# hawkn/emqx

Measured on AMD Instinct MI355X. Metric: topic matches/sec at 10M filters, higher is better.
Workload: dtype u8/u32; 1 GPU; c3: 10M mixed-wildcard filters incl. $share groups and '$SYS' exclusion; filters=10000002, topics_per_gpu_step=1000000, global_batch=1000000, parallelism=topic-sharded x1 (trie replicated), streams=3, distinct_batches=4, table_copies=1, outputs=pairs

## Files before the change

emqx_amd/build.py:

```python
from __future__ import annotations

import os
import subprocess
from pathlib import Path

PKG = Path(__file__).resolve().parent
ROOT = PKG.parent
CSRC = PKG / "csrc"

LIB_TMATCH = PKG / "libtmatch.so"
LIB_WORK = PKG / "libtmwork.so"
LIB_BENCH = PKG / "libtmbench.so"
LIB_ORACLE = ROOT / "oracle" / "liboracle.so"

ARCH = os.environ.get("TM_OFFLOAD_ARCH", "gfx950")


KERNEL_SOURCES = ("tm_kernels.hip", "tm_host.cpp", "tm_layout.h", "tm_dev.h")


def source_hash() -> str:
    import hashlib
    h = hashlib.sha256()
    for name in KERNEL_SOURCES:
        h.update(name.encode())
        h.update((CSRC / name).read_bytes())
    return h.hexdigest()[:16]


def _stale(out: Path, deps) -> bool:
    if not out.exists():
        return True
    t = out.stat().st_mtime
    return any(Path(d).stat().st_mtime > t for d in deps)


def _run(cmd, cwd=None):
    r = subprocess.run(cmd, cwd=cwd, capture_output=True, text=True)
    if r.returncode != 0:
        raise RuntimeError(f"build failed: {' '.join(map(str, cmd))}\n{r.stdout}\n{r.stderr}")


def build_tmatch(force: bool = False) -> Path:
    srcs = [CSRC / "tm_host.cpp", CSRC / "tm_kernels.hip"]
    deps = srcs + [CSRC / "tm_layout.h", CSRC / "tm_dev.h", ROOT / "include" / "tmatch.h"]
    if force or _stale(LIB_TMATCH, deps):
        tmp = LIB_TMATCH.with_suffix(".so.tmp")
        _run(["hipcc", "-O3", "-std=c++17", f"--offload-arch={ARCH}", "-fPIC", "-shared",
              "-Wall", "-Wno-unused-function", "-o", str(tmp)] + [str(s) for s in srcs])
        os.replace(tmp, LIB_TMATCH)
    return LIB_TMATCH


def build_variant(name: str, kernel_src: str | None = None, force: bool = False,
                  host_src: str | None = None) -> Path:
    out = PKG / "variants" / f"libtmatch_{name}.so"
    out.parent.mkdir(exist_ok=True)
    kern = Path(kernel_src) if kernel_src else CSRC / "tm_kernels.hip"
    srcs = [Path(host_src) if host_src else CSRC / "tm_host.cpp", kern]
    deps = srcs + [CSRC / "tm_layout.h", CSRC / "tm_dev.h", ROOT / "include" / "tmatch.h"]
    if force or _stale(out, deps):
        _run(["hipcc", "-O3", "-std=c++17", f"--offload-arch={ARCH}", "-fPIC", "-shared", "-Wall",
              "-Wno-unused-function", f"-I{CSRC}", "-o", str(out)] + [str(s) for s in srcs])
    return out


def build_work(force: bool = False) -> Path:
    src = CSRC / "workload.cpp"
    if force or _stale(LIB_WORK, [src]):
        tmp = LIB_WORK.with_suffix(".so.tmp")
        _run(["g++", "-O2", "-std=c++17", "-fPIC", "-shared", "-pthread", "-o", str(tmp), str(src)])
        os.replace(tmp, LIB_WORK)
    return LIB_WORK


def build_bench(force: bool = False) -> Path:
    src = CSRC / "hostbench.cpp"
    if force or _stale(LIB_BENCH, [src, ROOT / "include" / "tmatch.h"]):
        tmp = LIB_BENCH.with_suffix(".so.tmp")
        _run(["hipcc", "-O2", "-std=c++17", "-fPIC", "-shared", "-pthread", "-o", str(tmp), str(src), "-ldl"])
        os.replace(tmp, LIB_BENCH)
    return LIB_BENCH


def build_oracle(force: bool = False) -> Path:
    src = ROOT / "oracle" / "tm_oracle.c"
    if force or _stale(LIB_ORACLE, [src]):
        _run(["make", "-B" if force else "-s", "liboracle.so"], cwd=ROOT / "oracle")
    return LIB_ORACLE


def build_all(force: bool = False) -> None:
    build_tmatch(force)
    build_work(force)
    build_bench(force)
    build_oracle(force)


if __name__ == "__main__":
    build_all(force=True)
    print("built", LIB_TMATCH, LIB_WORK, LIB_ORACLE)
```

emqx_amd/csrc/tm_kernels.hip:

```cpp
#include "tm_dev.h"

#if defined(__HIP_DEVICE_COMPILE__) && !defined(__gfx950__)
#error "tm_kernels.hip: the tail tickets' ordering is argued for gfx950 only (see above)"
#endif

namespace tmx {


__device__ __forceinline__ uint4 ld4(const void *p) { return *reinterpret_cast<const uint4 *>(p); }
__device__ __forceinline__ uint4 ld4_once(const void *p) {
    typedef unsigned int u32x4 __attribute__((ext_vector_type(4)));
    const u32x4 v = __builtin_nontemporal_load(reinterpret_cast<const u32x4 *>(p));
    return make_uint4(v.x, v.y, v.z, v.w);
}

__device__ __forceinline__ uint32_t bloom_bit(const uint4 &n2, const uint4 &n3, uint32_t b) {
    const uint32_t j = b >> 5;
    const uint32_t w = j == 0 ? n2.z : j == 1 ? n2.w : j == 2 ? n3.x : j == 3 ? n3.y : j == 4 ? n3.z : n3.w;
    return (w >> (b & 31)) & 1u;
}

__device__ __forceinline__ uint32_t child_maybe(const DevIndex &ix, const uint4 &n1, const uint4 &n2, const uint4 &n3,
                                                uint32_t w, uint32_t h) {
    if ((n1.y & NLIT_MASK) >= WIDE_LIT)
        return n2.z == NONE ? 1u : w < ix.wcap ? (ix.wbits[n2.z + (w >> 5)] >> (w & 31)) & 1u : 0u;
    return bloom_bit(n2, n3, child_bit(h));
}

__device__ __forceinline__ bool child_alive(uint32_t lo, uint32_t hi, uint32_t lq, uint32_t L, uint32_t wq,
                                            uint32_t wq2) {
    const uint64_t m = (uint64_t)hi << 32 | lo;
    constexpr uint32_t AT_END = PSUM_HASH | PSUM_EXACT | PSUM_HDESC;
    if (lq == L) return (m & AT_END) != 0;
    if (m & PSUM_HASH) return true;
    if (wq != NONE && ((m >> (PSUM_BQ + psum_bit(child_hash(wq)))) & 1u)) return true;
    if (!(m & PSUM_PLUS)) return false;
    const uint32_t qq = (uint32_t)(m >> PSUM_QQ) & 15u;
    if (lq + 1 == L) return (qq & AT_END) != 0;
    if (qq & (PSUM_HASH | PSUM_PLUS)) return true;
    return wq2 != NONE && ((m >> (PSUM_BQQ + psum_bit(child_hash(wq2)))) & 1u);
}

__device__ __forceinline__ void pin(uint32_t &v) { asm volatile("" : "+v"(v)); }
__device__ __forceinline__ void pin(uint2 &v) { pin(v.x); pin(v.y); }
__device__ __forceinline__ void pin(uint4 &v) { pin(v.x); pin(v.y); pin(v.z); pin(v.w); }

struct WordAcc {
    uint32_t len, b0, b1;
    uint64_t start;
    __device__ __forceinline__ void reset(uint64_t s) {
        len = 0; b0 = b1 = 0; start = s;
    }
    __device__ __forceinline__ void push(uint32_t c) {
        uint32_t v = c << ((len & 3) * 8);
        if (len < 4) b0 |= v; else if (len < 8) b1 |= v;
        len++;
    }
};

struct GlobalSrc {
    const uint8_t *g;
    __device__ __forceinline__ uint4 ld16(uint64_t p) const { return ld4_once(g + p); }
    __device__ __forceinline__ uint32_t byte(uint64_t p) const { return g[p]; }
};
struct StagedSrc {
    const uint8_t *g;
    const uint4 *lds;
    uint64_t b0;
    bool staged;
    __device__ __forceinline__ uint4 ld16(uint64_t p) const {
        return staged ? lds[(uint32_t)(p - b0) >> 4] : ld4_once(g + p);
    }
    __device__ __forceinline__ uint32_t byte(uint64_t p) const {
        return staged ? reinterpret_cast<const uint8_t *>(lds)[(uint32_t)(p - b0)] : g[p];
    }
};

template <class Src>
__device__ bool bytes_eq(const uint8_t *a, const Src &src, uint64_t b, uint32_t n) {
    for (uint32_t i = 0; i < n; i++) if (a[i] != src.byte(b + i)) return false;
    return true;
}

template <class Src>
__device__ __forceinline__ uint64_t word_hash_dev(const WordAcc &w, const Src &src) {
    if (w.len <= VINL) return word_hash_short(w.b0, w.b1, w.len);
    uint64_t h = FNV_OFF;
    for (uint32_t i = 0; i < w.len; i++) h = (h ^ src.byte(w.start + i)) * FNV_PRIME;
    return word_hash_finish(h, w.len);
}

template <class Src>
__device__ uint32_t vocab_probe(const DevIndex &ix, uint32_t slot, uint32_t tag, uint32_t len, uint32_t b0,
                                uint32_t b1, const Src &src, uint64_t start) {
    for (;;) {
        const uint4 e = ld4(ix.vocab + slot);
        if (e.y == NONE) return NONE;
        if (e.x == tag) {
            if (len <= VINL) {
                if (e.z == b0 && e.w == b1) return e.y;
            } else if (e.w == len && bytes_eq(ix.wpool + e.z, src, start, len)) {
                return e.y;
            }
        }
        slot = (slot + 1) & ix.vmask;
    }
}

__device__ uint32_t vocab_probe_short(const DevIndex &ix, uint32_t slot, uint32_t tag, uint32_t b0, uint32_t b1) {
    for (;;) {
        const uint4 e = ld4(ix.vocab + slot);
        if (e.y == NONE) return NONE;
        if (e.x == tag && e.z == b0 && e.w == b1) return e.y;
        slot = (slot + 1) & ix.vmask;
    }
}

template <class Src>
__device__ uint32_t vocab_find(const DevIndex &ix, const WordAcc &w, const Src &src) {
    const uint64_t h = word_hash_dev(w, src);
    return vocab_probe(ix, (uint32_t)h & ix.vmask, vocab_tag(h, w.len), w.len, w.b0, w.b1, src, w.start);
}

__device__ __forceinline__ uint32_t ctab_find(const DevIndex &ix, uint32_t off, uint32_t mask, uint32_t wid,
                                              uint32_t h, uint32_t &slo, uint32_t &shi) {
    for (uint32_t s = h & mask;; s = (s + 1) & mask) {
        uint4 e = ld4(ix.ctab + off + s);
        pin(e);
        if (e.x == wid) { slo = e.z; shi = e.w; return e.y; }
        if (e.x == NONE) return NONE;
    }
}


template <int ML, bool LITE = false>
struct LdsStore {
    static constexpr uint32_t maxl = ML;
    static constexpr bool deferred = true;
    static constexpr bool cuts = ML > FAST_L;
    static constexpr bool need = ML > FAST_L || LITE;
    uint32_t *wid, *pend;
    uint8_t *len8;
    uint32_t stride;
    uint64_t mask;
    uint32_t pm;
    __device__ __forceinline__ void down(uint32_t l, bool via_plus) {
        if constexpr (cuts) pm = via_plus ? pm | (1u << l) : pm & ~(1u << l);
    }
    __device__ __forceinline__ void popped(uint32_t l) {
        if constexpr (cuts) pm &= (1u << (l - 1)) - 1u;
    }
    __device__ __forceinline__ void cut(uint32_t) {
        if constexpr (cuts) mask &= pm ? (1ull << (33u - __clz(pm))) - 1ull : 0ull;
    }
    __device__ __forceinline__ uint32_t get_wid(uint32_t l) const { return wid[l * stride]; }
    __device__ __forceinline__ void set_wid(uint32_t l, uint32_t w) { wid[l * stride] = w; }
    __device__ __forceinline__ void reset() { mask = 0; pm = 0; }
    __device__ __forceinline__ void put_word(uint32_t l, uint32_t b0, uint32_t b1, uint32_t len) {
        wid[l * stride] = b0; pend[l * stride] = b1; len8[l * stride] = (uint8_t)len;
    }
    __device__ __forceinline__ uint32_t word_b0(uint32_t l) const { return wid[l * stride]; }
    __device__ __forceinline__ uint32_t word_b1(uint32_t l) const { return pend[l * stride]; }
    __device__ __forceinline__ uint32_t word_len(uint32_t l) const { return len8[l * stride]; }
    __device__ __forceinline__ void push(uint32_t l, uint32_t node) {
        pend[l * stride] = node; mask |= 1ull << l;
    }
    __device__ __forceinline__ bool pop(uint32_t &l, uint32_t &node) {
        if (!mask) return false;
        l = 63u - (uint32_t)__clzll(mask);
        mask &= ~(1ull << l);
        node = pend[l * stride];
        return true;
    }
};

struct GlobalStore {
    static constexpr uint32_t maxl = MAX_LEVELS;
    static constexpr bool deferred = false;
    static constexpr bool cuts = true;
    static constexpr bool need = true;
    uint32_t *wid;
    uint2 *stk;
    uint8_t *plus_at;
    uint32_t top;
    __device__ __forceinline__ uint32_t get_wid(uint32_t l) const { return wid[l]; }
    __device__ __forceinline__ void set_wid(uint32_t l, uint32_t w) { wid[l] = w; }
    __device__ __forceinline__ void reset() { top = 0; }
    __device__ __forceinline__ void down(uint32_t l, bool via_plus) { plus_at[l] = via_plus; }
    __device__ __forceinline__ void popped(uint32_t l) { plus_at[l - 1] = 0; }
    __device__ void cut(uint32_t L) {
        int64_t q = (int64_t)L - 1;
        while (q >= 0 && !plus_at[q]) q--;
        while (top && (int64_t)stk[top - 1].x > q + 1) top--;
    }
    __device__ __forceinline__ void push(uint32_t l, uint32_t node) { stk[top++] = make_uint2(l, node); }
    __device__ __forceinline__ bool pop(uint32_t &l, uint32_t &node) {
        if (!top) return false;
        uint2 e = stk[--top]; l = e.x; node = e.y;
        return true;
    }
};


enum { RC_OK = 0, RC_BADARG = 1, RC_DEEP = 2 };

constexpr uint32_t VGROUP = 6;

template <class Src>
__device__ __noinline__ uint32_t count_slashes(const Src src, uint64_t p, uint64_t end) {
    uint32_t n = 0;
    for (; p < end; p += 64) {
        uint4 v[4];
#pragma unroll
        for (int c = 0; c < 4; c++) v[c] = p + 16 * c < end ? src.ld16(p + 16 * c) : make_uint4(0, 0, 0, 0);
#pragma unroll
        for (int c = 0; c < 4; c++) {
            const uint32_t w[4] = {v[c].x, v[c].y, v[c].z, v[c].w};
            const uint64_t q = p + 16 * c;
            const int k1 = q >= end ? 0 : end - q < 16 ? (int)(end - q) : 16;
#pragma unroll
            for (int j = 0; j < 4; j++) {
                const uint32_t x = w[j] ^ 0x2F2F2F2Fu;
                uint32_t nz = (((x & 0x7F7F7F7Fu) + 0x7F7F7F7Fu) | x) & 0x80808080u;
                const int valid = k1 - 4 * j;
                if (valid < 4) nz |= valid <= 0 ? 0x80808080u : 0x80808080u << (8 * valid);
                n += 4 - __popc(nz);
            }
        }
    }
    return n;
}

template <class S, class Src>
__device__ int tokenize(const DevIndex &ix, const Src &src, uint64_t beg, uint64_t end, S &st,
                        uint32_t &L, bool &dollar, uint64_t &xh, bool &all_found) {
    uint64_t longmask = 0;
    all_found = true; dollar = false; xh = FNV_OFF;
    const uint64_t p0 = beg & ~15ull;
    const uint4 z = make_uint4(0, 0, 0, 0);
    const uint4 c0 = p0 < end ? src.ld16(p0) : z;
    const uint4 c1 = p0 + 16 < end ? src.ld16(p0 + 16) : z;
    if constexpr (S::deferred) {
        constexpr bool NEED = S::need;
        uint32_t lev = 0, len = 0, b0 = 0, b1 = 0;
        uint64_t ws = beg;
        bool bad = false;
        auto park = [&]() {
            if (lev < S::maxl) {
                if (len <= VINL) st.put_word(lev, b0, b1, len);
                else st.put_word(lev, len, (uint32_t)(ws - beg), 255);
            } else if constexpr (NEED) {
                bad |= len == 1 && ((b0 & 0xFFu) == '+' || (b0 & 0xFFu) == '#');
            }
            lev++;
        };
        uint32_t ci = 0;
        uint64_t p = p0;
        uint4 ra = c0, rb = c1;
        for (; p < end; p += 16, ci++) {
            if (!NEED && lev > S::maxl) break;
            uint4 v;
            if constexpr (NEED) {
                v = ra; ra = rb;
                rb = p + 32 < end ? src.ld16(p + 32) : z;
            } else {
                v = ci == 0 ? c0 : ci == 1 ? c1 : src.ld16(p);
            }
            const uint32_t k0 = p < beg ? (uint32_t)(beg - p) : 0;
            const uint32_t k1 = end - p < 16 ? (uint32_t)(end - p) : 16;
#pragma unroll
            for (uint32_t k = 0; k < 16; k++) {
                if (k < k0 || k >= k1) continue;
                const uint32_t word = k < 4 ? v.x : k < 8 ? v.y : k < 12 ? v.z : v.w;
                const uint32_t c = (word >> ((k & 3) * 8)) & 0xFFu;
                if (c == '/') {
                    park();
                    len = 0; b0 = 0; b1 = 0; ws = p + k + 1;
                } else {
                    const uint32_t sh = (len & 3) * 8;
                    b0 |= len < 4 ? c << sh : 0u;
                    b1 |= len - 4 < 4 ? c << sh : 0u;
                    len++;
                }
            }
        }
        if (!NEED && p < end) {
            const bool any = ix.xlen_max <= S::maxl && ix.depth + 2 <= (uint32_t)MID_L &&
                             end - beg < (uint64_t)MAX_LEVELS;
            L = any ? lev + 1 : lev + 1 + count_slashes(src, p, end);
            return RC_DEEP;
        }
        park();
        if (lev > (NEED ? MAX_LEVELS : S::maxl)) { L = lev; return RC_DEEP; }
        L = lev;
        for (uint32_t l = 0; l < L && l < S::maxl; l++) {
            const uint32_t n = st.word_len(l), c = st.word_b0(l) & 0xFFu;
            bad |= n == 1 && (c == '+' || c == '#');
        }
        if (bad) return RC_BADARG;
        if constexpr (NEED) {
            const uint32_t Lw = need_levels(ix, L);
            if (Lw + (Lw < L ? 2 : 0) > S::maxl) return RC_DEEP;
            L |= Lw << 24;
        }
        dollar = st.word_len(0) == 255 ? src.byte(beg) == '$' : st.word_len(0) >= 1 && (st.word_b0(0) & 0xFFu) == '$';
        for (uint32_t l = 0; l < (S::need ? L >> 24 : L); l++) {
            if (st.word_len(l) != 255) continue;
            WordAcc w; w.reset(beg + st.word_b1(l)); w.len = st.word_b0(l);
            st.set_wid(l, vocab_find(ix, w, src));
            longmask |= 1ull << l;
        }
    } else {
        WordAcc w; w.reset(beg);
        uint32_t lev = 0;
        auto finish = [&]() -> int {
            if (w.len == 1 && (w.b0 == '+' || w.b0 == '#')) return RC_BADARG;
            if (lev >= S::maxl) return RC_DEEP;
            if (lev == 0 && w.len >= 1 && (w.b0 & 0xFF) == '$') dollar = true;
            st.set_wid(lev, vocab_find(ix, w, src));
            lev++;
            return RC_OK;
        };
        uint32_t ci = 0;
        for (uint64_t p = p0; p < end; p += 16, ci++) {
            const uint4 v = ci == 0 ? c0 : ci == 1 ? c1 : src.ld16(p);
            const uint32_t k0 = p < beg ? (uint32_t)(beg - p) : 0;
            const uint32_t k1 = end - p < 16 ? (uint32_t)(end - p) : 16;
            for (uint32_t k = k0; k < k1; k++) {
                const uint32_t word = k < 4 ? v.x : k < 8 ? v.y : k < 12 ? v.z : v.w;
                const uint32_t c = (word >> ((k & 3) * 8)) & 0xFFu;
                if (c == '/') {
                    int rc = finish();
                    if (rc) return rc;
                    w.reset(p + k + 1);
                } else {
                    w.push(c);
                }
            }
        }
        int rc = finish();
        if (rc) return rc;
        L = lev;
    }
    if constexpr (S::deferred) {
        for (uint32_t base = 0; base < (S::need ? L >> 24 : L); base += VGROUP) {
            uint4 e[VGROUP];
            uint32_t tg[VGROUP];
            bool use[VGROUP];
#pragma unroll
            for (uint32_t k = 0; k < VGROUP; k++) {
                const uint32_t l = base + k;
                use[k] = l < (S::need ? L >> 24 : L) && !((longmask >> l) & 1);
                const uint32_t ls = use[k] ? l : 0;
                const uint32_t len = st.word_len(ls);
                const uint64_t h = word_hash_short(st.word_b0(ls), st.word_b1(ls), len);
                tg[k] = vocab_tag(h, len);
                e[k] = ld4(ix.vocab + (use[k] ? ((uint32_t)h & ix.vmask) : 0u));
            }
#pragma unroll
            for (uint32_t k = 0; k < VGROUP; k++) {
                const uint32_t l = use[k] ? base + k : 0;
                const uint32_t b0 = st.word_b0(l), b1 = st.word_b1(l);
                const bool hit = e[k].x == tg[k] && e[k].z == b0 && e[k].w == b1;
                uint32_t wid = e[k].y == NONE ? NONE : hit ? e[k].y : NONE - 1;
                pin(wid);
                if (use[k]) {
                    if (wid == NONE - 1) {
                        const uint32_t len = st.word_len(l);
                        const uint64_t h = word_hash_short(b0, b1, len);
                        wid = vocab_probe_short(ix, ((uint32_t)h + 1) & ix.vmask, tg[k], b0, b1);
                    }
                    st.set_wid(l, wid);
                }
            }
        }
    }
    if constexpr (S::deferred && S::need) {
      const uint32_t Lw = L >> 24;
      L &= 0xFFFFFFu;
      if (Lw < L) {
        st.set_wid(Lw, NONE);
        st.set_wid(Lw + 1, NONE);
        all_found = false;
        return RC_OK;
      }
    }
    for (uint32_t l = 0; l < L; l++) {
        const uint32_t wid = st.get_wid(l);
        all_found &= wid != NONE;
        xh = seq_hash_step(xh, wid);
    }
    xh = seq_hash_finish(xh, L);
    return RC_OK;
}

__device__ __forceinline__ int tail_list(const DevIndex &ix, uint32_t nl) {
    return nl <= MAX_LEVELS && need_levels(ix, nl) <= MID_L ? L_MID : L_DEEP;
}

template <class S>
__device__ void exact_find(const DevIndex &ix, uint64_t xh, uint32_t L, const S &st, uint32_t slot, uint32_t f,
                           uint32_t &off, uint32_t &cnt) {
    cnt = 0; off = 0;
    const uint32_t fp = exact_fp(xh);
    for (;;) {
        if (f == 0) return;
        if (f == fp) {
            const uint4 *e = reinterpret_cast<const uint4 *>(ix.exact + slot);
            uint4 a = e[0], b = e[1], c = e[2], d = e[3];
            pin(a); pin(b); pin(c); pin(d);
            if (a.x == (uint32_t)xh && a.y == (uint32_t)(xh >> 32) && a.z == L) {
                bool eq = true;
                if (L <= XINL) {
                    const uint32_t iw[XINL] = {b.z, b.w, c.x, c.y, c.z, c.w, d.x, d.y, d.z, d.w};
#pragma unroll
                    for (uint32_t l = 0; l < XINL; l++)
                        if (l < L) eq &= iw[l] == st.get_wid(l);
                } else {
                    for (uint32_t l = 0; l < L && eq; l++) eq = ix.wseq[b.y + l] == st.get_wid(l);
                }
                if (eq) { off = a.w; cnt = b.x; return; }
            }
        }
        slot = (slot + 1) & ix.xmask;
        f = ix.xfp[slot];
    }
}


enum { DFS_DONE = 0, DFS_STOP = 1, DFS_REROUTE = 2 };
template <class S, class EM>
__device__ int dfs(const DevIndex &ix, uint32_t L, bool dollar, S &st, EM &em) {
    uint32_t cur = ROOT, l = 0;
    for (;;) {
        const uint4 *np = reinterpret_cast<const uint4 *>(ix.nodes + cur);
        const uint4 n0 = np[0];
        const uint4 n1 = np[1];
        const uint4 n2 = np[2];
        const uint4 n3 = np[3];
        const bool droot = dollar && l == 0;
        const uint32_t w = l < L ? st.get_wid(l) : NONE;
        uint32_t inl = n2.x == w ? n3.x : n2.y == w ? n3.y : n2.z == w ? n3.z : n2.w == w ? n3.w : NONE;
        pin(inl);
        if (l == L) {
            if (!em(n0.w, n1.x)) return DFS_STOP;
            if (!droot && !em(n0.y, n0.z)) return DFS_STOP;
            if (n1.y & NLIT_HDESC) {
                if constexpr (!S::cuts) return DFS_REROUTE;
                st.cut(L);
            }
        } else {
            uint32_t lit = NONE;
            if (w != NONE) {
                if ((n1.y & NLIT_MASK) <= KINL) {
                    lit = inl;
                } else {
                    const uint32_t h = child_hash(w);
                    if (child_maybe(ix, n1, n2, n3, w, h) & 1u) {
                        uint32_t slo, shi;
                        lit = ctab_find(ix, n2.x, n2.y, w, h, slo, shi);
                        if (lit != NONE && !child_alive(slo, shi, l + 1, L, l + 1 < L ? st.get_wid(l + 1) : NONE,
                                                        l + 2 < L ? st.get_wid(l + 2) : NONE))
                            lit = NONE;
                    }
                }
            }
            if (!droot && !em(n0.y, n0.z)) return DFS_STOP;
            uint32_t plus = droot || (n1.y & NLIT_HDESC) ? NONE : n0.x;
            if (plus != NONE && !child_alive(n1.z, n1.w, l + 1, L, l + 1 < L ? st.get_wid(l + 1) : NONE,
                                             l + 2 < L ? st.get_wid(l + 2) : NONE))
                plus = NONE;
            if (plus != NONE) {
                if (lit != NONE) st.push(l + 1, lit);
                st.down(l, true);
                cur = plus; l++;
                continue;
            }
            if (lit != NONE) {
                st.down(l, false);
                cur = lit; l++;
                continue;
            }
        }
        if (!st.pop(l, cur)) return DFS_DONE;
        st.popped(l);
    }
}


struct RangeEmit {
    uint2 r[RCAP];
    uint32_t cnt, nr;
    __device__ __forceinline__ bool operator()(uint32_t off, uint32_t n) {
        if (n) {
#pragma unroll
            for (uint32_t i = 0; i < RCAP; i++)
                if (nr == i) r[i] = make_uint2(off, n);
            nr++; cnt += n & RUN_CNT;
        }
        return true;
    }
    __device__ __forceinline__ void store(uint2 *rng, uint64_t n, uint64_t t) const {
#pragma unroll
        for (uint32_t i = 0; i < RCAP; i++)
            if (i < nr) __builtin_nontemporal_store((uint64_t)r[i].x | ((uint64_t)r[i].y << 32),
                                                    reinterpret_cast<uint64_t *>(rng) + (uint64_t)i * n + t);
    }
};

struct DirectEmit {
    const uint32_t *vals;
    uint32_t *out;
    uint64_t pos, cap;
    __device__ __forceinline__ bool operator()(uint32_t off, uint32_t n) {
        const uint32_t c = n & RUN_CNT;
        for (uint32_t i = 0; i < c; i++, pos++)
            if (pos < cap) out[pos] = (n & RUN_INLINE) ? off : vals[off + i];
        return true;
    }
};

struct FirstEmit {
    const uint32_t *vals;
    uint32_t v;
    bool found;
    __device__ __forceinline__ bool operator()(uint32_t off, uint32_t n) {
        if (n) { v = (n & RUN_INLINE) ? off : vals[off]; found = true; return false; }
        return true;
    }
};

template <class S, class EM, class Src>
__device__ __forceinline__ int match_topic(const DevIndex &ix, const Src &src, uint64_t beg, uint64_t end, S &st,
                                           EM &em, uint32_t *levels = nullptr) {
    uint32_t L = 0; bool dollar, allf; uint64_t xh;
    int rc = tokenize(ix, src, beg, end, st, L, dollar, xh, allf);
    if (levels) *levels = L;
    if (rc) return rc;
    st.reset();
    const uint32_t xslot = (uint32_t)xh & ix.xmask;
    const uint32_t xf = allf ? ix.xfp[xslot] : 0;
    const int d = dfs(ix, L, dollar, st, em);
    if (d == DFS_STOP) return RC_OK;
    if (d == DFS_REROUTE) {
        if (levels) *levels = L;
        return RC_DEEP;
    }
    if (allf) {
        uint32_t xoff, xcnt;
        exact_find(ix, xh, L, st, xslot, xf, xoff, xcnt);
        em(xoff, xcnt);
    }
    return RC_OK;
}

enum { MODE_COUNT = 0, MODE_FIRST = 1 };

struct Outs {
    uint8_t *err;
    uint32_t *first_val;
    uint8_t *first_found;
};

__device__ __forceinline__ void list_push_wave(const Workspace &ws, uint64_t n, int k, uint32_t t) {
    const uint32_t lane = threadIdx.x & 63;
    for (int j = 0; j < L_COUNT; j++) {
        if (!__ballot(k >= 0)) break;
        const uint64_t m = __ballot(k == j);
        if (!m) continue;
        const uint32_t leader = (uint32_t)__ffsll((unsigned long long)m) - 1;
        uint32_t base = 0;
        if (lane == leader) base = atomicAdd(&ws.list_n[j], (uint32_t)__popcll(m));
        base = (uint32_t)__shfl((int)base, (int)leader, 64);
        if (k == j) ws.lists[(uint64_t)j * n + base + (uint32_t)__popcll(m & ((1ull << lane) - 1))] = t;
    }
}

__device__ __forceinline__ void list_push(const Workspace &ws, uint64_t n, int k, uint32_t t) {
    uint32_t i = atomicAdd(&ws.list_n[k], 1u);
    ws.lists[(uint64_t)k * n + i] = t;
}

template <int MODE, class S>
__device__ int run_topic(const DevIndex &ix, const Workspace &ws, uint64_t n, const uint8_t *blob,
                         const uint64_t *offs, uint64_t t, S &st, const Outs &o, uint32_t *hits,
                         int *ovf = nullptr) {
    const uint64_t beg = offs[t], end = offs[t + 1];
    if (MODE == MODE_COUNT) {
        RangeEmit em;
        em.cnt = 0; em.nr = 0;
        uint32_t levels;
        int rc = match_topic(ix, GlobalSrc{blob}, beg, end, st, em, &levels);
        const bool toolong = rc == RC_DEEP && S::maxl == MAX_LEVELS;
        if (rc == RC_DEEP && !toolong) { *hits = levels; return rc; }
        if (rc != RC_OK) { em.cnt = 0; em.nr = 0; }
        __builtin_nontemporal_store(em.cnt, ws.cnt + t);
        __builtin_nontemporal_store(em.nr, ws.nr + t);
        em.store(ws.rng, n, t);
        __builtin_nontemporal_store((uint8_t)(rc == RC_BADARG ? 1 : (toolong ? 2 : 0)), o.err + t);
        if (em.nr > RCAP) {
            const int k = S::maxl <= MID_L ? L_OVF_MID : L_OVF_DEEP;
            if (ovf) *ovf = k; else list_push(ws, n, k, (uint32_t)t);
        }
        *hits = em.cnt;
        return rc;
    } else {
        FirstEmit em{ix.vals, 0, false};
        uint32_t levels;
        int rc = match_topic(ix, GlobalSrc{blob}, beg, end, st, em, &levels);
        const bool toolong = rc == RC_DEEP && S::maxl == MAX_LEVELS;
        if (rc == RC_DEEP && !toolong) { *hits = levels; return rc; }
        o.first_val[t] = toolong ? 0 : em.v;
        o.first_found[t] = rc == RC_BADARG ? 2 : (toolong ? 3 : (em.found ? 1 : 0));
        *hits = 0;
        return rc;
// ... 1668 lines not shown
```

emqx_amd/csrc/tm_layout.h:

```cpp
#pragma once
#include <stdint.h>

#if defined(__HIPCC__)
#define TM_HD __host__ __device__ __forceinline__
#else
#define TM_HD inline
#endif

namespace tmx {

constexpr uint32_t NONE = 0xFFFFFFFFu;
constexpr uint32_t ROOT = 0;
constexpr uint32_t VINL = 8;
constexpr uint32_t XINL = 10;

struct alignas(16) VocabEntry {
    uint32_t tag;
    uint32_t wid;
    uint32_t b0, b1;
};

struct alignas(16) CSlot {
    uint32_t wid;
    uint32_t child;
    uint32_t sum_lo, sum_hi;
};

constexpr uint32_t KINL = 4;

constexpr uint32_t WIDE_LIT = 256;

struct alignas(64) Node {
    uint32_t plus;
    uint32_t hash_off, hash_cnt;
    uint32_t exact_off, exact_cnt;
    uint32_t nlit;
    uint32_t psum_lo, psum_hi;
    uint32_t kw[KINL];
    uint32_t kc[KINL];
};

constexpr uint32_t NLIT_HDESC = 0x80000000u;
constexpr uint32_t NLIT_MASK = 0x7FFFFFFFu;

constexpr uint32_t PSUM_HASH = 1u, PSUM_EXACT = 2u, PSUM_PLUS = 4u, PSUM_HDESC = 8u;
constexpr uint32_t PSUM_QQ = 4, PSUM_BQ = 8, PSUM_BQQ = 36, PSUM_BLOOM = 28;

struct alignas(16) ExactEntry {
    uint32_t h_lo, h_hi;
    uint32_t nlev;
    uint32_t val_off, val_cnt;
    uint32_t seq_off;
    uint32_t wids[XINL];
};

constexpr uint32_t RUN_INLINE = 0x80000000u;
constexpr uint32_t RUN_CNT = 0x7FFFFFFFu;

static_assert(sizeof(VocabEntry) == 16, "vocab entry");
static_assert(sizeof(CSlot) == 16, "child slot");
static_assert(sizeof(Node) == 64, "node");
static_assert(sizeof(ExactEntry) == 64, "exact entry");


TM_HD uint64_t mix64(uint64_t x) {
    x ^= x >> 30; x *= 0xbf58476d1ce4e5b9ull;
    x ^= x >> 27; x *= 0x94d049bb133111ebull;
    x ^= x >> 31;
    return x;
}

constexpr uint64_t FNV_OFF = 0xcbf29ce484222325ull;
constexpr uint64_t FNV_PRIME = 0x100000001b3ull;

TM_HD uint64_t word_hash_short(uint32_t b0, uint32_t b1, uint32_t len) {
    return mix64((((uint64_t)b1 << 32) | b0) + 0x9e3779b97f4a7c15ull * (len + 1));
}
TM_HD uint64_t word_hash_finish(uint64_t fnv, uint32_t len) { return mix64(fnv ^ ((uint64_t)len << 56)); }

TM_HD uint32_t vocab_tag(uint64_t h, uint32_t len) {
    return ((uint32_t)(h >> 32) & 0xFFFFFF00u) | (len < 255 ? len : 255);
}

TM_HD uint32_t child_hash(uint32_t wid) { return (uint32_t)mix64((uint64_t)wid * 0x9e3779b97f4a7c15ull + 1); }
TM_HD uint32_t child_bit(uint32_t h) { return ((h >> 16) * 192u) >> 16; }
TM_HD uint32_t psum_bit(uint32_t h) { return ((h >> 16) * PSUM_BLOOM) >> 16; }
TM_HD uint32_t &bloom_word(Node &n, uint32_t j) { return j < 2 ? n.kw[2 + j] : n.kc[j - 2]; }

TM_HD uint16_t exact_fp(uint64_t h) { return (uint16_t)((h >> 48) | 1u); }

TM_HD uint64_t seq_hash_step(uint64_t h, uint32_t wid) { return (h ^ wid) * FNV_PRIME; }
TM_HD uint64_t seq_hash_finish(uint64_t h, uint32_t nlev) { return mix64(h + 0x9e3779b97f4a7c15ull * (nlev + 1)); }

}
```

Before: 4.477 billion topic matches/s.

## Tokenize topics with SWAR slash masks and use a cheaper 32-bit child hash

Replaces the per-byte unrolled tokenizer loop in the deferred path with a new scan_levels helper. It builds a 16-bit slash mask per 16-byte chunk with SWAR arithmetic and iterates over the set bits, extracting each word with funnel shifts instead of branching on every byte. It also swaps the 64-bit mix64-based child_hash for a 32-bit integer hash. The hash change alters child bloom bit positions, so trie construction and device lookup must both use the new function. The variable-trip loop over mask bits may also diverge more across lanes than the fixed unrolled byte loop.

```diff
diff --git a/emqx_amd/build.py b/emqx_amd/build.py
--- a/emqx_amd/build.py
+++ b/emqx_amd/build.py
@@ -16,7 +16,7 @@
 ARCH = os.environ.get("TM_OFFLOAD_ARCH", "gfx950")
 
 
-KERNEL_SOURCES = ("tm_kernels.hip", "tm_host.cpp", "tm_layout.h", "tm_dev.h")
+KERNEL_SOURCES = ("tm_kernels.hip", "tm_host.cpp", "tm_layout.h", "tm_dev.h", "tm_scan.h")
 
 
 def source_hash() -> str:
@@ -43,7 +43,7 @@
 
 def build_tmatch(force: bool = False) -> Path:
     srcs = [CSRC / "tm_host.cpp", CSRC / "tm_kernels.hip"]
-    deps = srcs + [CSRC / "tm_layout.h", CSRC / "tm_dev.h", ROOT / "include" / "tmatch.h"]
+    deps = srcs + [CSRC / "tm_layout.h", CSRC / "tm_dev.h", CSRC / "tm_scan.h", ROOT / "include" / "tmatch.h"]
     if force or _stale(LIB_TMATCH, deps):
         tmp = LIB_TMATCH.with_suffix(".so.tmp")
         _run(["hipcc", "-O3", "-std=c++17", f"--offload-arch={ARCH}", "-fPIC", "-shared",
@@ -58,7 +58,7 @@
     out.parent.mkdir(exist_ok=True)
     kern = Path(kernel_src) if kernel_src else CSRC / "tm_kernels.hip"
     srcs = [Path(host_src) if host_src else CSRC / "tm_host.cpp", kern]
-    deps = srcs + [CSRC / "tm_layout.h", CSRC / "tm_dev.h", ROOT / "include" / "tmatch.h"]
+    deps = srcs + [CSRC / "tm_layout.h", CSRC / "tm_dev.h", CSRC / "tm_scan.h", ROOT / "include" / "tmatch.h"]
     if force or _stale(out, deps):
         _run(["hipcc", "-O3", "-std=c++17", f"--offload-arch={ARCH}", "-fPIC", "-shared", "-Wall",
               "-Wno-unused-function", f"-I{CSRC}", "-o", str(out)] + [str(s) for s in srcs])
diff --git a/emqx_amd/csrc/tm_kernels.hip b/emqx_amd/csrc/tm_kernels.hip
--- a/emqx_amd/csrc/tm_kernels.hip
+++ b/emqx_amd/csrc/tm_kernels.hip
@@ -1,4 +1,5 @@
 #include "tm_dev.h"
+#include "tm_scan.h"
 
 #if defined(__HIP_DEVICE_COMPILE__) && !defined(__gfx950__)
 #error "tm_kernels.hip: the tail tickets' ordering is argued for gfx950 only (see above)"
@@ -236,61 +237,17 @@
                         uint32_t &L, bool &dollar, uint64_t &xh, bool &all_found) {
     uint64_t longmask = 0;
     all_found = true; dollar = false; xh = FNV_OFF;
-    const uint64_t p0 = beg & ~15ull;
-    const uint4 z = make_uint4(0, 0, 0, 0);
-    const uint4 c0 = p0 < end ? src.ld16(p0) : z;
-    const uint4 c1 = p0 + 16 < end ? src.ld16(p0 + 16) : z;
     if constexpr (S::deferred) {
         constexpr bool NEED = S::need;
-        uint32_t lev = 0, len = 0, b0 = 0, b1 = 0;
-        uint64_t ws = beg;
-        bool bad = false;
-        auto park = [&]() {
-            if (lev < S::maxl) {
-                if (len <= VINL) st.put_word(lev, b0, b1, len);
-                else st.put_word(lev, len, (uint32_t)(ws - beg), 255);
-            } else if constexpr (NEED) {
-                bad |= len == 1 && ((b0 & 0xFFu) == '+' || (b0 & 0xFFu) == '#');
-            }
-            lev++;
-        };
-        uint32_t ci = 0;
-        uint64_t p = p0;
-        uint4 ra = c0, rb = c1;
-        for (; p < end; p += 16, ci++) {
-            if (!NEED && lev > S::maxl) break;
-            uint4 v;
-            if constexpr (NEED) {
-                v = ra; ra = rb;
-                rb = p + 32 < end ? src.ld16(p + 32) : z;
-            } else {
-                v = ci == 0 ? c0 : ci == 1 ? c1 : src.ld16(p);
-            }
-            const uint32_t k0 = p < beg ? (uint32_t)(beg - p) : 0;
-            const uint32_t k1 = end - p < 16 ? (uint32_t)(end - p) : 16;
-#pragma unroll
-            for (uint32_t k = 0; k < 16; k++) {
-                if (k < k0 || k >= k1) continue;
-                const uint32_t word = k < 4 ? v.x : k < 8 ? v.y : k < 12 ? v.z : v.w;
-                const uint32_t c = (word >> ((k & 3) * 8)) & 0xFFu;
-                if (c == '/') {
-                    park();
-                    len = 0; b0 = 0; b1 = 0; ws = p + k + 1;
-                } else {
-                    const uint32_t sh = (len & 3) * 8;
-                    b0 |= len < 4 ? c << sh : 0u;
-                    b1 |= len - 4 < 4 ? c << sh : 0u;
-                    len++;
-                }
-            }
-        }
-        if (!NEED && p < end) {
+        const ScanOut sc = scan_levels<NEED>(src, beg, end, st);
+        const uint32_t lev = sc.lev;
+        bool bad = sc.bad;
+        if (sc.early) {
             const bool any = ix.xlen_max <= S::maxl && ix.depth + 2 <= (uint32_t)MID_L &&
                              end - beg < (uint64_t)MAX_LEVELS;
-            L = any ? lev + 1 : lev + 1 + count_slashes(src, p, end);
+            L = any ? lev + 1 : lev + 1 + count_slashes(src, sc.p, end);
             return RC_DEEP;
         }
-        park();
         if (lev > (NEED ? MAX_LEVELS : S::maxl)) { L = lev; return RC_DEEP; }
         L = lev;
         for (uint32_t l = 0; l < L && l < S::maxl; l++) {
@@ -311,6 +268,10 @@
             longmask |= 1ull << l;
         }
     } else {
+        const uint64_t p0 = beg & ~15ull;
+        const uint4 z = make_uint4(0, 0, 0, 0);
+        const uint4 c0 = p0 < end ? src.ld16(p0) : z;
+        const uint4 c1 = p0 + 16 < end ? src.ld16(p0 + 16) : z;
         WordAcc w; w.reset(beg);
         uint32_t lev = 0;
         auto finish = [&]() -> int {
diff --git a/emqx_amd/csrc/tm_layout.h b/emqx_amd/csrc/tm_layout.h
--- a/emqx_amd/csrc/tm_layout.h
+++ b/emqx_amd/csrc/tm_layout.h
@@ -82,7 +82,13 @@
     return ((uint32_t)(h >> 32) & 0xFFFFFF00u) | (len < 255 ? len : 255);
 }
 
-TM_HD uint32_t child_hash(uint32_t wid) { return (uint32_t)mix64((uint64_t)wid * 0x9e3779b97f4a7c15ull + 1); }
+TM_HD uint32_t child_hash(uint32_t wid) {
+    uint32_t x = wid + 0x9e3779b9u;
+    x ^= x >> 16; x *= 0x7feb352du;
+    x ^= x >> 15; x *= 0x846ca68bu;
+    x ^= x >> 16;
+    return x;
+}
 TM_HD uint32_t child_bit(uint32_t h) { return ((h >> 16) * 192u) >> 16; }
 TM_HD uint32_t psum_bit(uint32_t h) { return ((h >> 16) * PSUM_BLOOM) >> 16; }
 TM_HD uint32_t &bloom_word(Node &n, uint32_t j) { return j < 2 ? n.kw[2 + j] : n.kc[j - 2]; }
diff --git a/emqx_amd/csrc/tm_scan.h b/emqx_amd/csrc/tm_scan.h
--- /dev/null
+++ b/emqx_amd/csrc/tm_scan.h
@@ -0,0 +1,95 @@
+#pragma once
+#include "tm_layout.h"
+
+namespace tmx {
+
+struct ScanOut {
+    uint32_t lev;
+    bool bad;
+    bool early;
+    uint64_t p;
+};
+
+TM_HD uint32_t slash_mask16(uint32_t w0, uint32_t w1, uint32_t w2, uint32_t w3) {
+    auto z = [](uint32_t w) {
+        const uint32_t x = w ^ 0x2F2F2F2Fu;
+        return ~((((x & 0x7F7F7F7Fu) + 0x7F7F7F7Fu) | x)) & 0x80808080u;
+    };
+    auto pack8 = [](uint32_t a, uint32_t b) {
+        uint32_t t = (a >> 7) | (b >> 3);
+        t |= t >> 7;
+        t |= t >> 14;
+        return t & 0xFFu;
+    };
+    return pack8(z(w0), z(w1)) | pack8(z(w2), z(w3)) << 8;
+}
+
+template <bool NEED, class Src, class St>
+TM_HD ScanOut scan_levels(const Src &src, uint64_t beg, uint64_t end, St &st) {
+    using V = decltype(src.ld16(beg));
+    V z = V(); z.x = 0; z.y = 0; z.z = 0; z.w = 0;
+    const uint64_t p0 = beg & ~15ull;
+    const V c0 = p0 < end ? src.ld16(p0) : z;
+    const V c1 = p0 + 16 < end ? src.ld16(p0 + 16) : z;
+    uint32_t lev = 0, len = 0, ws = 0;
+    uint64_t acc = 0;
+    bool bad = false;
+    uint32_t ci = 0;
+    uint64_t p = p0;
+    V ra = c0, rb = c1;
+    for (; p < end; p += 16, ci++) {
+        if (!NEED && lev > St::maxl) break;
+        V v;
+        if (NEED) {
+            v = ra; ra = rb;
+            rb = p + 32 < end ? src.ld16(p + 32) : z;
+        } else {
+            v = ci == 0 ? c0 : ci == 1 ? c1 : src.ld16(p);
+        }
+        const uint32_t k0 = p < beg ? (uint32_t)(beg - p) : 0;
+        const uint32_t k1 = end - p < 16 ? (uint32_t)(end - p) : 16;
+        const uint32_t rel = (uint32_t)(p - beg);
+        uint32_t m = (slash_mask16(v.x, v.y, v.z, v.w) & ((1u << k1) - (1u << k0))) | 1u << k1;
+        uint32_t s = k0;
+        for (;;) {
+            const uint32_t e = (uint32_t)__builtin_ctz(m);
+            m &= m - 1;
+            const uint32_t n = e - s, d = s >> 2, sh = (s & 3) * 8;
+            const uint32_t x0 = d == 0 ? v.x : d == 1 ? v.y : d == 2 ? v.z : v.w;
+            const uint32_t x1 = d == 0 ? v.y : d == 1 ? v.z : d == 2 ? v.w : 0u;
+            const uint32_t x2 = d == 0 ? v.z : d == 1 ? v.w : 0u;
+            const uint32_t lo = (uint32_t)(((uint64_t)x1 << 32 | x0) >> sh);
+            const uint32_t hi = (uint32_t)(((uint64_t)x2 << 32 | x1) >> sh);
+            uint64_t x = (uint64_t)hi << 32 | lo;
+            if (n < VINL) x &= (1ull << (8 * n)) - 1ull;
+            if (len < VINL) acc |= x << (8 * len);
+            len += n;
+            if (e == k1) break;
+            if (lev < St::maxl) {
+                if (len <= VINL) st.put_word(lev, (uint32_t)acc, (uint32_t)(acc >> 32), len);
+                else st.put_word(lev, len, ws, 255);
+            } else if (NEED) {
+                bad |= len == 1 && ((acc & 0xFFu) == '+' || (acc & 0xFFu) == '#');
+            }
+            lev++;
+            len = 0; acc = 0; s = e + 1; ws = rel + s;
+        }
+    }
+    ScanOut o;
+    o.p = p;
+    o.early = !NEED && p < end;
+    if (!o.early) {
+        if (lev < St::maxl) {
+            if (len <= VINL) st.put_word(lev, (uint32_t)acc, (uint32_t)(acc >> 32), len);
+            else st.put_word(lev, len, ws, 255);
+        } else if (NEED) {
+            bad |= len == 1 && ((acc & 0xFFu) == '+' || (acc & 0xFFu) == '#');
+        }
+        lev++;
+    }
+    o.lev = lev;
+    o.bad = bad;
+    return o;
+}
+
+}
```

New measurement: 4.557 billion topic matches/s (median of 6 runs). 1.8% higher.
